# lucidrains/naturalspeech2-pytorch

Measured on NVIDIA H100. Metric: denoiser-steps/sec, higher is better.
Workload: dtype bf16

## Files before the change

naturalspeech2_pytorch_b200/csrc/attn.cu:

```cuda
#include "ptx.cuh"
#include "philox.cuh"
#include "host_common.h"
#include "../../include/ns2_b200.h"

namespace ns2 {

namespace attn {
constexpr int BQ = 128;
constexpr int BKV = 128;
constexpr int DH = 64;
constexpr int KVS = 3;
constexpr int Q_BYTES = BQ * DH * 2;
constexpr int KV_BYTES = BKV * DH * 2;
constexpr int OFF_Q = 0;
constexpr int OFF_K = OFF_Q + Q_BYTES;
constexpr int OFF_V = OFF_K + KVS * KV_BYTES;
constexpr int OFF_BAR = OFF_V + KVS * KV_BYTES;
constexpr int SMEM_BYTES = OFF_BAR + 256;
constexpr int THREADS = 384;
}

struct AttnDev {
  CUtensorMap tmQ, tmK, tmV;
  __nv_bfloat16* out;
  long long o_rs, o_bs;
  int q_len, kv_len;
  float scale_log2e;
  float* lse;
  DropoutDev drop;
  const int* kv_lens;
};

__device__ __forceinline__ float ex2_approx(float x) {
  float y;
  asm("ex2.approx.ftz.f32 %0, %1;" : "=f"(y) : "f"(x));
  return y;
}

__device__ __forceinline__ float keep_if(float x, uint32_t bits, int n) { return (bits >> n) & 1u ? x : 0.f; }

template <bool DROPOUT, bool RAGGED>
__global__ void __launch_bounds__(attn::THREADS, 1) attn_fwd_kernel(const __grid_constant__ AttnDev p) {
  static_assert(!(DROPOUT && RAGGED), "no dropout variant of the key-padding kernel");
  using namespace attn;
  extern __shared__ __align__(1024) uint8_t smem[];
  uint64_t* bars = reinterpret_cast<uint64_t*>(smem + OFF_BAR);
  uint64_t* q_full = bars + 0;
  uint64_t* kv_full = bars + 1;
  uint64_t* kv_empty = bars + 1 + KVS;

  const int warp = threadIdx.x >> 5, lane = threadIdx.x & 31;
  const int q0 = blockIdx.x * BQ;
  const int head = blockIdx.y;
  const int b = blockIdx.z;
  const int kv_len_b = RAGGED ? min(max(__ldg(p.kv_lens + b), 1), p.kv_len) : 0;
#define NS2_ATTN_KV_LEN (RAGGED ? kv_len_b : p.kv_len)
  const int T = (NS2_ATTN_KV_LEN + BKV - 1) / BKV;

  if (threadIdx.x == 0) {
    if ((smem_u32(smem) & 1023u) != 0) __trap();
    tma_prefetch_desc(&p.tmQ);
    tma_prefetch_desc(&p.tmK);
    tma_prefetch_desc(&p.tmV);
    mbar_init(smem_u32(q_full), 1);
    for (int i = 0; i < KVS; ++i) {
      mbar_init(smem_u32(&kv_full[i]), 1);
      mbar_init(smem_u32(&kv_empty[i]), 8);
    }
    fence_barrier_init();
  }
  __syncthreads();

  if (warp < 4) {
    asm volatile("setmaxnreg.dec.sync.aligned.u32 40;");
    if (warp == 0 && lane == 0) {
      mbar_arrive_expect_tx(smem_u32(q_full), Q_BYTES);
      tma_load_3d(smem_u32(smem + OFF_Q), &p.tmQ, smem_u32(q_full), head * DH, q0, b);
      for (int j = 0; j < T; ++j) {
        const int st = j % KVS;
        const uint32_t ph = (j / KVS) & 1;
        mbar_wait(smem_u32(&kv_empty[st]), ph ^ 1);
        const uint32_t fb = smem_u32(&kv_full[st]);
        mbar_arrive_expect_tx(fb, 2 * KV_BYTES);
        tma_load_3d(smem_u32(smem + OFF_K + st * KV_BYTES), &p.tmK, fb, head * DH, j * BKV, b);
        tma_load_3d(smem_u32(smem + OFF_V + st * KV_BYTES), &p.tmV, fb, head * DH, j * BKV, b);
      }
    }
  } else {
    asm volatile("setmaxnreg.inc.sync.aligned.u32 232;");
    const int w = (warp >> 2) - 1;
    const int r0 = 64 * w + 16 * (warp & 3) + (lane >> 2);
    const int c2 = 2 * (lane & 3);
    const float c = p.scale_log2e;
    float o_acc[DH / 2];
#pragma unroll
    for (int i = 0; i < DH / 2; ++i) o_acc[i] = 0.f;
    float m_run[2] = {-INFINITY, -INFINITY}, l_run[2] = {0.f, 0.f};
    const uint64_t dq = gmma_desc_sw128(smem_u32(smem + OFF_Q + w * (64 * 128)), 16, 1024);
    mbar_wait(smem_u32(q_full), 0);

    for (int j = 0; j < T; ++j) {
      const int st = j % KVS;
      mbar_wait(smem_u32(&kv_full[st]), (j / KVS) & 1);
      float s[BKV / 2];
      uint32_t keep[2];
      {
        const uint64_t dk = gmma_desc_sw128(smem_u32(smem + OFF_K + st * KV_BYTES), 16, 1024);
        wgmma_fence();
#pragma unroll
        for (int k = 0; k < DH / 16; ++k) wgmma_bf16_ss_n128<0, 0>(s, dq + 2 * k, dk + 2 * k, k > 0 ? 1u : 0u);
        wgmma_commit();
        if constexpr (DROPOUT) {
          const uint32_t cq = philox_attn_index(q0 + r0), cbh = b * gridDim.y + head, th = p.drop.threshold;
#pragma unroll
          for (int h = 0; h < 2; ++h) {
            keep[h] = 0u;
#pragma unroll 1
            for (int kk = 0; kk < 4; ++kk)
#pragma unroll
              for (int t = 0; t < 2; ++t) {
                const Philox4 r = philox4x32_10(philox_attn_index(j * BKV + 16 * (4 * h + kk) + c2 + t), cq, cbh,
                                                p.drop.site, p.drop.key0, p.drop.key1);
                const int n = 8 * kk + t;
                keep[h] |= (r.x >= th ? 1u : 0u) << n | (r.y >= th ? 1u : 0u) << (n + 4) |
                           (r.z >= th ? 1u : 0u) << (n + 2) | (r.w >= th ? 1u : 0u) << (n + 6);
              }
          }
        }
        wgmma_wait<0>();
        wgmma_hold(s);
      }
      const int valid = NS2_ATTN_KV_LEN - j * BKV;
      if (valid < BKV) {
#pragma unroll
        for (int jj = 0; jj < BKV / 8; ++jj)
#pragma unroll
          for (int e = 0; e < 4; ++e)
            if (8 * jj + c2 + (e & 1) >= valid) s[4 * jj + e] = -INFINITY;
      }
      float a[2], m_new[2];
#pragma unroll
      for (int i = 0; i < 2; ++i) {
        float m = -INFINITY;
#pragma unroll
        for (int jj = 0; jj < BKV / 8; ++jj) m = fmaxf(m, fmaxf(s[4 * jj + 2 * i], s[4 * jj + 2 * i + 1]));
        m = fmaxf(m, __shfl_xor_sync(0xffffffffu, m, 1));
        m = fmaxf(m, __shfl_xor_sync(0xffffffffu, m, 2));
        m_new[i] = fmaxf(m_run[i], m * c);
        a[i] = ex2_approx(m_run[i] - m_new[i]);
        m_run[i] = m_new[i];
        l_run[i] *= a[i];
      }
#pragma unroll
      for (int jj = 0; jj < DH / 8; ++jj) {
        o_acc[4 * jj + 0] *= a[0];
        o_acc[4 * jj + 1] *= a[0];
        o_acc[4 * jj + 2] *= a[1];
        o_acc[4 * jj + 3] *= a[1];
      }
      uint32_t pa[BKV / 16][4];
#pragma unroll
      for (int jj = 0; jj < BKV / 8; ++jj) {
        const float p0 = ex2_approx(fmaf(s[4 * jj + 0], c, -m_new[0]));
        const float p1 = ex2_approx(fmaf(s[4 * jj + 1], c, -m_new[0]));
        const float p2 = ex2_approx(fmaf(s[4 * jj + 2], c, -m_new[1]));
        const float p3 = ex2_approx(fmaf(s[4 * jj + 3], c, -m_new[1]));
        l_run[0] += p0 + p1;
        l_run[1] += p2 + p3;
        if constexpr (DROPOUT) {
          const uint32_t kb = keep[jj >> 3];
          const int n = (4 * jj) & 31;
          pa[jj >> 1][(jj & 1) * 2 + 0] = pack_bf16x2(keep_if(p0, kb, n), keep_if(p1, kb, n + 1));
          pa[jj >> 1][(jj & 1) * 2 + 1] = pack_bf16x2(keep_if(p2, kb, n + 2), keep_if(p3, kb, n + 3));
        } else {
          pa[jj >> 1][(jj & 1) * 2 + 0] = pack_bf16x2(p0, p1);
          pa[jj >> 1][(jj & 1) * 2 + 1] = pack_bf16x2(p2, p3);
        }
      }
      {
        const uint32_t vbase = smem_u32(smem + OFF_V + st * KV_BYTES);
        wgmma_fence();
#pragma unroll
        for (int k = 0; k < BKV / 16; ++k)
          wgmma_bf16_rs_n64<1>(o_acc, pa[k], gmma_desc_sw128(vbase + k * 2048, 1024, 1024), 1u);
        wgmma_commit();
        wgmma_wait<0>();
        wgmma_hold(o_acc);
      }
      __syncwarp();
      if (lane == 0) mbar_arrive(smem_u32(&kv_empty[st]));
    }

#pragma unroll
    for (int i = 0; i < 2; ++i) {
      float l = l_run[i];
      l += __shfl_xor_sync(0xffffffffu, l, 1);
      l += __shfl_xor_sync(0xffffffffu, l, 2);
      const int qrow = q0 + r0 + 8 * i;
      if (qrow < p.q_len) {
        const float inv = DROPOUT ? p.drop.scale / l : 1.0f / l;
        if (p.lse != nullptr && (lane & 3) == 0)
          p.lse[(static_cast<long long>(b) * gridDim.y + head) * p.q_len + qrow] = m_run[i] + log2f(l);
        __nv_bfloat16* op = p.out + static_cast<long long>(b) * p.o_bs + static_cast<long long>(qrow) * p.o_rs +
                            head * DH + c2;
#pragma unroll
        for (int jj = 0; jj < DH / 8; ++jj)
          *reinterpret_cast<uint32_t*>(op + 8 * jj) =
              pack_bf16x2(o_acc[4 * jj + 2 * i] * inv, o_acc[4 * jj + 2 * i + 1] * inv);
      }
    }
  }
#undef NS2_ATTN_KV_LEN
}

}

using namespace ns2;

extern "C" int ns2_attn_fwd(const ns2_attn_args* a, ns2_stream_t stream_) {
  NS2_REQUIRE(a != nullptr, "attn_fwd: NULL args");
  const ns2_dropout* d = a->dropout;
  DropoutDev drop;
  NS2_REQUIRE(d == nullptr || make_dropout_dev(d->seed, d->site, d->p, &drop), "attn_fwd: dropout p=%g is not in [0, 1)",
              static_cast<double>(d->p));
  const bool dropout = d != nullptr && d->p != 0.0f;
  NS2_REQUIRE(!(dropout && a->kv_lens), "attn_fwd: kv_lens with dropout p > 0 is not supported");
  NS2_REQUIRE(a->q && a->k && a->v && a->out, "attn_fwd: NULL pointer");
  NS2_REQUIRE(a->dim_head == 64, "attn_fwd: dim_head=%d, only 64 is supported", a->dim_head);
  NS2_REQUIRE(a->batches > 0 && a->heads > 0 && a->q_len > 0 && a->kv_len > 0, "attn_fwd: empty problem");
  NS2_REQUIRE(a->o_row_stride % 8 == 0 && a->o_batch_stride % 8 == 0 &&
                  (reinterpret_cast<uintptr_t>(a->out) & 15) == 0,
              "attn_fwd: out must be 16-byte aligned with strides multiple of 8");
  const cudaStream_t stream = static_cast<cudaStream_t>(stream_);
  AttnDev dev;
  memset(&dev, 0, sizeof(dev));
  const uint32_t box[3] = {64, attn::BQ, 1};
  const uint32_t box_kv[3] = {64, attn::BKV, 1};
  {
    const uint64_t dims[3] = {(uint64_t)a->heads * 64, (uint64_t)a->q_len, (uint64_t)a->batches};
    const uint64_t str[3] = {2, (uint64_t)a->q_row_stride * 2, (uint64_t)a->q_batch_stride * 2};
    int rc = make_tmap_16bit(&dev.tmQ, a->q, 3, dims, str, box);
    if (rc != kOk) return rc;
  }
  {
    const uint64_t dims[3] = {(uint64_t)a->heads * 64, (uint64_t)a->kv_len, (uint64_t)a->batches};
    const uint64_t strk[3] = {2, (uint64_t)a->k_row_stride * 2, (uint64_t)a->k_batch_stride * 2};
    const uint64_t strv[3] = {2, (uint64_t)a->v_row_stride * 2, (uint64_t)a->v_batch_stride * 2};
    int rc = make_tmap_16bit(&dev.tmK, a->k, 3, dims, strk, box_kv);
    if (rc != kOk) return rc;
    rc = make_tmap_16bit(&dev.tmV, a->v, 3, dims, strv, box_kv);
    if (rc != kOk) return rc;
  }
  dev.out = reinterpret_cast<__nv_bfloat16*>(a->out);
  dev.o_rs = a->o_row_stride;
  dev.o_bs = a->o_batch_stride;
  dev.q_len = a->q_len;
  dev.kv_len = a->kv_len;
  dev.scale_log2e = a->scale * 1.4426950408889634f;
  dev.lse = a->lse;
  dim3 grid((a->q_len + attn::BQ - 1) / attn::BQ, a->heads, a->batches);
  if (a->kv_lens != nullptr) {
    dev.kv_lens = a->kv_lens;
    NS2_CUDA_CHECK(set_max_smem_once(attn_fwd_kernel<false, true>, attn::SMEM_BYTES));
    attn_fwd_kernel<false, true><<<grid, attn::THREADS, attn::SMEM_BYTES, stream>>>(dev);
  } else if (!dropout) {
    NS2_CUDA_CHECK(set_max_smem_once(attn_fwd_kernel<false, false>, attn::SMEM_BYTES));
    attn_fwd_kernel<false, false><<<grid, attn::THREADS, attn::SMEM_BYTES, stream>>>(dev);
  } else {
    dev.drop = drop;
    NS2_CUDA_CHECK(set_max_smem_once(attn_fwd_kernel<true, false>, attn::SMEM_BYTES));
    attn_fwd_kernel<true, false><<<grid, attn::THREADS, attn::SMEM_BYTES, stream>>>(dev);
  }
  return launched(1);
}
```

Before: 65.78.

## Make attention forward kernel persistent with cross-tile Q/KV prefetch

Turns the flash-attention forward kernel into a persistent kernel: the grid is capped at the SM count and each CTA loops over (q-tile, head, batch) work items. The producer warp keeps a global KV stage counter so the K/V ring buffer carries across tiles, and a new q_empty barrier lets it load the next Q tile once consumers finish their last QK^T. This is meant to hide per-CTA launch, prologue and tail latency and to overlap the next tile's loads with the current tile's epilogue. In exchange the item-to-CTA mapping is static round-robin, which can leave tail imbalance when items have uneven KV lengths.

New measurement: 66.50, median of 6. 1.01x the previous value.

```diff
diff --git a/naturalspeech2_pytorch_b200/csrc/attn.cu b/naturalspeech2_pytorch_b200/csrc/attn.cu
--- a/naturalspeech2_pytorch_b200/csrc/attn.cu
+++ b/naturalspeech2_pytorch_b200/csrc/attn.cu
@@ -25,6 +25,7 @@
   __nv_bfloat16* out;
   long long o_rs, o_bs;
   int q_len, kv_len;
+  int q_tiles, heads, num_items;
   float scale_log2e;
   float* lse;
   DropoutDev drop;
@@ -48,14 +49,18 @@
   uint64_t* q_full = bars + 0;
   uint64_t* kv_full = bars + 1;
   uint64_t* kv_empty = bars + 1 + KVS;
+  uint64_t* q_empty = bars + 1 + 2 * KVS;
 
   const int warp = threadIdx.x >> 5, lane = threadIdx.x & 31;
-  const int q0 = blockIdx.x * BQ;
-  const int head = blockIdx.y;
-  const int b = blockIdx.z;
-  const int kv_len_b = RAGGED ? min(max(__ldg(p.kv_lens + b), 1), p.kv_len) : 0;
+  int q0, head, b, kv_len_b, T;
+  auto item = [&](int it) {
+    q0 = (it % p.q_tiles) * BQ;
+    head = (it / p.q_tiles) % p.heads;
+    b = it / (p.q_tiles * p.heads);
+    kv_len_b = RAGGED ? min(max(__ldg(p.kv_lens + b), 1), p.kv_len) : 0;
+    T = ((RAGGED ? kv_len_b : p.kv_len) + BKV - 1) / BKV;
+  };
 #define NS2_ATTN_KV_LEN (RAGGED ? kv_len_b : p.kv_len)
-  const int T = (NS2_ATTN_KV_LEN + BKV - 1) / BKV;
 
   if (threadIdx.x == 0) {
     if ((smem_u32(smem) & 1023u) != 0) __trap();
@@ -67,6 +72,7 @@
       mbar_init(smem_u32(&kv_full[i]), 1);
       mbar_init(smem_u32(&kv_empty[i]), 8);
     }
+    mbar_init(smem_u32(q_empty), 8);
     fence_barrier_init();
   }
   __syncthreads();
@@ -74,16 +80,21 @@
   if (warp < 4) {
     asm volatile("setmaxnreg.dec.sync.aligned.u32 40;");
     if (warp == 0 && lane == 0) {
-      mbar_arrive_expect_tx(smem_u32(q_full), Q_BYTES);
-      tma_load_3d(smem_u32(smem + OFF_Q), &p.tmQ, smem_u32(q_full), head * DH, q0, b);
-      for (int j = 0; j < T; ++j) {
-        const int st = j % KVS;
-        const uint32_t ph = (j / KVS) & 1;
-        mbar_wait(smem_u32(&kv_empty[st]), ph ^ 1);
-        const uint32_t fb = smem_u32(&kv_full[st]);
-        mbar_arrive_expect_tx(fb, 2 * KV_BYTES);
-        tma_load_3d(smem_u32(smem + OFF_K + st * KV_BYTES), &p.tmK, fb, head * DH, j * BKV, b);
-        tma_load_3d(smem_u32(smem + OFF_V + st * KV_BYTES), &p.tmV, fb, head * DH, j * BKV, b);
+      uint32_t n = 0, kt = 0;
+      for (int it = blockIdx.x; it < p.num_items; it += gridDim.x, ++n) {
+        item(it);
+        mbar_wait(smem_u32(q_empty), (n & 1) ^ 1);
+        mbar_arrive_expect_tx(smem_u32(q_full), Q_BYTES);
+        tma_load_3d(smem_u32(smem + OFF_Q), &p.tmQ, smem_u32(q_full), head * DH, q0, b);
+        for (int j = 0; j < T; ++j, ++kt) {
+          const int st = kt % KVS;
+          const uint32_t ph = (kt / KVS) & 1;
+          mbar_wait(smem_u32(&kv_empty[st]), ph ^ 1);
+          const uint32_t fb = smem_u32(&kv_full[st]);
+          mbar_arrive_expect_tx(fb, 2 * KV_BYTES);
+          tma_load_3d(smem_u32(smem + OFF_K + st * KV_BYTES), &p.tmK, fb, head * DH, j * BKV, b);
+          tma_load_3d(smem_u32(smem + OFF_V + st * KV_BYTES), &p.tmV, fb, head * DH, j * BKV, b);
+        }
       }
     }
   } else {
@@ -92,121 +103,129 @@
     const int r0 = 64 * w + 16 * (warp & 3) + (lane >> 2);
     const int c2 = 2 * (lane & 3);
     const float c = p.scale_log2e;
-    float o_acc[DH / 2];
-#pragma unroll
-    for (int i = 0; i < DH / 2; ++i) o_acc[i] = 0.f;
-    float m_run[2] = {-INFINITY, -INFINITY}, l_run[2] = {0.f, 0.f};
     const uint64_t dq = gmma_desc_sw128(smem_u32(smem + OFF_Q + w * (64 * 128)), 16, 1024);
-    mbar_wait(smem_u32(q_full), 0);
-
-    for (int j = 0; j < T; ++j) {
-      const int st = j % KVS;
-      mbar_wait(smem_u32(&kv_full[st]), (j / KVS) & 1);
-      float s[BKV / 2];
-      uint32_t keep[2];
-      {
-        const uint64_t dk = gmma_desc_sw128(smem_u32(smem + OFF_K + st * KV_BYTES), 16, 1024);
-        wgmma_fence();
-#pragma unroll
-        for (int k = 0; k < DH / 16; ++k) wgmma_bf16_ss_n128<0, 0>(s, dq + 2 * k, dk + 2 * k, k > 0 ? 1u : 0u);
-        wgmma_commit();
-        if constexpr (DROPOUT) {
-          const uint32_t cq = philox_attn_index(q0 + r0), cbh = b * gridDim.y + head, th = p.drop.threshold;
-#pragma unroll
-          for (int h = 0; h < 2; ++h) {
-            keep[h] = 0u;
+    uint32_t n = 0, kt = 0;
+    for (int it = blockIdx.x; it < p.num_items; it += gridDim.x, ++n) {
+      item(it);
+      float o_acc[DH / 2];
+#pragma unroll
+      for (int i = 0; i < DH / 2; ++i) o_acc[i] = 0.f;
+      float m_run[2] = {-INFINITY, -INFINITY}, l_run[2] = {0.f, 0.f};
+      mbar_wait(smem_u32(q_full), n & 1);
+
+      for (int j = 0; j < T; ++j, ++kt) {
+        const int st = kt % KVS;
+        mbar_wait(smem_u32(&kv_full[st]), (kt / KVS) & 1);
+        float s[BKV / 2];
+        uint32_t keep[2];
+        {
+          const uint64_t dk = gmma_desc_sw128(smem_u32(smem + OFF_K + st * KV_BYTES), 16, 1024);
+          wgmma_fence();
+#pragma unroll
+          for (int k = 0; k < DH / 16; ++k) wgmma_bf16_ss_n128<0, 0>(s, dq + 2 * k, dk + 2 * k, k > 0 ? 1u : 0u);
+          wgmma_commit();
+          if constexpr (DROPOUT) {
+            const uint32_t cq = philox_attn_index(q0 + r0), cbh = b * p.heads + head, th = p.drop.threshold;
+#pragma unroll
+            for (int h = 0; h < 2; ++h) {
+              keep[h] = 0u;
 #pragma unroll 1
-            for (int kk = 0; kk < 4; ++kk)
-#pragma unroll
-              for (int t = 0; t < 2; ++t) {
-                const Philox4 r = philox4x32_10(philox_attn_index(j * BKV + 16 * (4 * h + kk) + c2 + t), cq, cbh,
-                                                p.drop.site, p.drop.key0, p.drop.key1);
-                const int n = 8 * kk + t;
-                keep[h] |= (r.x >= th ? 1u : 0u) << n | (r.y >= th ? 1u : 0u) << (n + 4) |
-                           (r.z >= th ? 1u : 0u) << (n + 2) | (r.w >= th ? 1u : 0u) << (n + 6);
-              }
+              for (int kk = 0; kk < 4; ++kk)
+#pragma unroll
+                for (int t = 0; t < 2; ++t) {
+                  const Philox4 r = philox4x32_10(philox_attn_index(j * BKV + 16 * (4 * h + kk) + c2 + t), cq, cbh,
+                                                  p.drop.site, p.drop.key0, p.drop.key1);
+                  const int n = 8 * kk + t;
+                  keep[h] |= (r.x >= th ? 1u : 0u) << n | (r.y >= th ? 1u : 0u) << (n + 4) |
+                             (r.z >= th ? 1u : 0u) << (n + 2) | (r.w >= th ? 1u : 0u) << (n + 6);
+                }
+            }
           }
-        }
-        wgmma_wait<0>();
-        wgmma_hold(s);
+          wgmma_wait<0>();
+          wgmma_hold(s);
+        }
+        if (j == T - 1) {
+          __syncwarp();
+          if (lane == 0) mbar_arrive(smem_u32(q_empty));
+        }
+        const int valid = NS2_ATTN_KV_LEN - j * BKV;
+        if (valid < BKV) {
+#pragma unroll
+          for (int jj = 0; jj < BKV / 8; ++jj)
+#pragma unroll
+            for (int e = 0; e < 4; ++e)
+              if (8 * jj + c2 + (e & 1) >= valid) s[4 * jj + e] = -INFINITY;
+        }
+        float a[2], m_new[2];
+#pragma unroll
+        for (int i = 0; i < 2; ++i) {
+          float m = -INFINITY;
+#pragma unroll
+          for (int jj = 0; jj < BKV / 8; ++jj) m = fmaxf(m, fmaxf(s[4 * jj + 2 * i], s[4 * jj + 2 * i + 1]));
+          m = fmaxf(m, __shfl_xor_sync(0xffffffffu, m, 1));
+          m = fmaxf(m, __shfl_xor_sync(0xffffffffu, m, 2));
+          m_new[i] = fmaxf(m_run[i], m * c);
+          a[i] = ex2_approx(m_run[i] - m_new[i]);
+          m_run[i] = m_new[i];
+          l_run[i] *= a[i];
+        }
+#pragma unroll
+        for (int jj = 0; jj < DH / 8; ++jj) {
+          o_acc[4 * jj + 0] *= a[0];
+          o_acc[4 * jj + 1] *= a[0];
+          o_acc[4 * jj + 2] *= a[1];
+          o_acc[4 * jj + 3] *= a[1];
+        }
+        uint32_t pa[BKV / 16][4];
+#pragma unroll
+        for (int jj = 0; jj < BKV / 8; ++jj) {
+          const float p0 = ex2_approx(fmaf(s[4 * jj + 0], c, -m_new[0]));
+          const float p1 = ex2_approx(fmaf(s[4 * jj + 1], c, -m_new[0]));
+          const float p2 = ex2_approx(fmaf(s[4 * jj + 2], c, -m_new[1]));
+          const float p3 = ex2_approx(fmaf(s[4 * jj + 3], c, -m_new[1]));
+          l_run[0] += p0 + p1;
+          l_run[1] += p2 + p3;
+          if constexpr (DROPOUT) {
+            const uint32_t kb = keep[jj >> 3];
+            const int n = (4 * jj) & 31;
+            pa[jj >> 1][(jj & 1) * 2 + 0] = pack_bf16x2(keep_if(p0, kb, n), keep_if(p1, kb, n + 1));
+            pa[jj >> 1][(jj & 1) * 2 + 1] = pack_bf16x2(keep_if(p2, kb, n + 2), keep_if(p3, kb, n + 3));
+          } else {
+            pa[jj >> 1][(jj & 1) * 2 + 0] = pack_bf16x2(p0, p1);
+            pa[jj >> 1][(jj & 1) * 2 + 1] = pack_bf16x2(p2, p3);
+          }
+        }
+        {
+          const uint32_t vbase = smem_u32(smem + OFF_V + st * KV_BYTES);
+          wgmma_fence();
+#pragma unroll
+          for (int k = 0; k < BKV / 16; ++k)
+            wgmma_bf16_rs_n64<1>(o_acc, pa[k], gmma_desc_sw128(vbase + k * 2048, 1024, 1024), 1u);
+          wgmma_commit();
+          wgmma_wait<0>();
+          wgmma_hold(o_acc);
+        }
+        __syncwarp();
+        if (lane == 0) mbar_arrive(smem_u32(&kv_empty[st]));
       }
-      const int valid = NS2_ATTN_KV_LEN - j * BKV;
-      if (valid < BKV) {
-#pragma unroll
-        for (int jj = 0; jj < BKV / 8; ++jj)
-#pragma unroll
-          for (int e = 0; e < 4; ++e)
-            if (8 * jj + c2 + (e & 1) >= valid) s[4 * jj + e] = -INFINITY;
-      }
-      float a[2], m_new[2];
+
 #pragma unroll
       for (int i = 0; i < 2; ++i) {
-        float m = -INFINITY;
-#pragma unroll
-        for (int jj = 0; jj < BKV / 8; ++jj) m = fmaxf(m, fmaxf(s[4 * jj + 2 * i], s[4 * jj + 2 * i + 1]));
-        m = fmaxf(m, __shfl_xor_sync(0xffffffffu, m, 1));
-        m = fmaxf(m, __shfl_xor_sync(0xffffffffu, m, 2));
-        m_new[i] = fmaxf(m_run[i], m * c);
-        a[i] = ex2_approx(m_run[i] - m_new[i]);
-        m_run[i] = m_new[i];
-        l_run[i] *= a[i];
-      }
-#pragma unroll
-      for (int jj = 0; jj < DH / 8; ++jj) {
-        o_acc[4 * jj + 0] *= a[0];
-        o_acc[4 * jj + 1] *= a[0];
-        o_acc[4 * jj + 2] *= a[1];
-        o_acc[4 * jj + 3] *= a[1];
-      }
-      uint32_t pa[BKV / 16][4];
-#pragma unroll
-      for (int jj = 0; jj < BKV / 8; ++jj) {
-        const float p0 = ex2_approx(fmaf(s[4 * jj + 0], c, -m_new[0]));
-        const float p1 = ex2_approx(fmaf(s[4 * jj + 1], c, -m_new[0]));
-        const float p2 = ex2_approx(fmaf(s[4 * jj + 2], c, -m_new[1]));
-        const float p3 = ex2_approx(fmaf(s[4 * jj + 3], c, -m_new[1]));
-        l_run[0] += p0 + p1;
-        l_run[1] += p2 + p3;
-        if constexpr (DROPOUT) {
-          const uint32_t kb = keep[jj >> 3];
-          const int n = (4 * jj) & 31;
-          pa[jj >> 1][(jj & 1) * 2 + 0] = pack_bf16x2(keep_if(p0, kb, n), keep_if(p1, kb, n + 1));
-          pa[jj >> 1][(jj & 1) * 2 + 1] = pack_bf16x2(keep_if(p2, kb, n + 2), keep_if(p3, kb, n + 3));
-        } else {
-          pa[jj >> 1][(jj & 1) * 2 + 0] = pack_bf16x2(p0, p1);
-          pa[jj >> 1][(jj & 1) * 2 + 1] = pack_bf16x2(p2, p3);
-        }
-      }
-      {
-        const uint32_t vbase = smem_u32(smem + OFF_V + st * KV_BYTES);
-        wgmma_fence();
-#pragma unroll
-        for (int k = 0; k < BKV / 16; ++k)
-          wgmma_bf16_rs_n64<1>(o_acc, pa[k], gmma_desc_sw128(vbase + k * 2048, 1024, 1024), 1u);
-        wgmma_commit();
-        wgmma_wait<0>();
-        wgmma_hold(o_acc);
-      }
-      __syncwarp();
-      if (lane == 0) mbar_arrive(smem_u32(&kv_empty[st]));
-    }
-
-#pragma unroll
-    for (int i = 0; i < 2; ++i) {
-      float l = l_run[i];
-      l += __shfl_xor_sync(0xffffffffu, l, 1);
-      l += __shfl_xor_sync(0xffffffffu, l, 2);
-      const int qrow = q0 + r0 + 8 * i;
-      if (qrow < p.q_len) {
-        const float inv = DROPOUT ? p.drop.scale / l : 1.0f / l;
-        if (p.lse != nullptr && (lane & 3) == 0)
-          p.lse[(static_cast<long long>(b) * gridDim.y + head) * p.q_len + qrow] = m_run[i] + log2f(l);
-        __nv_bfloat16* op = p.out + static_cast<long long>(b) * p.o_bs + static_cast<long long>(qrow) * p.o_rs +
-                            head * DH + c2;
-#pragma unroll
-        for (int jj = 0; jj < DH / 8; ++jj)
-          *reinterpret_cast<uint32_t*>(op + 8 * jj) =
-              pack_bf16x2(o_acc[4 * jj + 2 * i] * inv, o_acc[4 * jj + 2 * i + 1] * inv);
+        float l = l_run[i];
+        l += __shfl_xor_sync(0xffffffffu, l, 1);
+        l += __shfl_xor_sync(0xffffffffu, l, 2);
+        const int qrow = q0 + r0 + 8 * i;
+        if (qrow < p.q_len) {
+          const float inv = DROPOUT ? p.drop.scale / l : 1.0f / l;
+          if (p.lse != nullptr && (lane & 3) == 0)
+            p.lse[(static_cast<long long>(b) * p.heads + head) * p.q_len + qrow] = m_run[i] + log2f(l);
+          __nv_bfloat16* op = p.out + static_cast<long long>(b) * p.o_bs + static_cast<long long>(qrow) * p.o_rs +
+                              head * DH + c2;
+#pragma unroll
+          for (int jj = 0; jj < DH / 8; ++jj)
+            *reinterpret_cast<uint32_t*>(op + 8 * jj) =
+                pack_bf16x2(o_acc[4 * jj + 2 * i] * inv, o_acc[4 * jj + 2 * i + 1] * inv);
+        }
       }
     }
   }
@@ -258,7 +277,11 @@
   dev.kv_len = a->kv_len;
   dev.scale_log2e = a->scale * 1.4426950408889634f;
   dev.lse = a->lse;
-  dim3 grid((a->q_len + attn::BQ - 1) / attn::BQ, a->heads, a->batches);
+  dev.q_tiles = (a->q_len + attn::BQ - 1) / attn::BQ;
+  dev.heads = a->heads;
+  NS2_REQUIRE(static_cast<long long>(dev.q_tiles) * a->heads * a->batches <= INT32_MAX, "attn_fwd: too many tiles");
+  dev.num_items = dev.q_tiles * a->heads * a->batches;
+  const int grid = dev.num_items < num_sms() ? dev.num_items : num_sms();
   if (a->kv_lens != nullptr) {
     dev.kv_lens = a->kv_lens;
     NS2_CUDA_CHECK(set_max_smem_once(attn_fwd_kernel<false, true>, attn::SMEM_BYTES));
```

## Make attention kernel persistent with ping-pong warpgroups and overlapped PV GEMM

Applied to the files above, without the earlier changes.

Turns the attention forward kernel into a persistent kernel launched with one CTA per SM that loops over query tiles. The producer now double-buffers Q tiles and uses four KV stages. The two consumer warpgroups take turns on the tensor cores through named barriers. Each iteration issues the previous block's P·V wgmma together with the current QK^T wgmma, so one warpgroup's softmax can overlap the other's matrix work. This adds synchronisation complexity, more shared memory, and register pressure from carrying P across iterations.

Measured after the change: 65.81 before, 66.91 after (median of 6 runs). +1.7%, better.

```diff
diff --git a/naturalspeech2_pytorch_b200/csrc/attn.cu b/naturalspeech2_pytorch_b200/csrc/attn.cu
--- a/naturalspeech2_pytorch_b200/csrc/attn.cu
+++ b/naturalspeech2_pytorch_b200/csrc/attn.cu
@@ -9,15 +9,17 @@
 constexpr int BQ = 128;
 constexpr int BKV = 128;
 constexpr int DH = 64;
-constexpr int KVS = 3;
+constexpr int KVS = 4;
+constexpr int QS = 2;
 constexpr int Q_BYTES = BQ * DH * 2;
 constexpr int KV_BYTES = BKV * DH * 2;
 constexpr int OFF_Q = 0;
-constexpr int OFF_K = OFF_Q + Q_BYTES;
+constexpr int OFF_K = OFF_Q + QS * Q_BYTES;
 constexpr int OFF_V = OFF_K + KVS * KV_BYTES;
 constexpr int OFF_BAR = OFF_V + KVS * KV_BYTES;
 constexpr int SMEM_BYTES = OFF_BAR + 256;
 constexpr int THREADS = 384;
+constexpr int TURN_BAR = 1;
 }
 
 struct AttnDev {
@@ -25,6 +27,7 @@
   __nv_bfloat16* out;
   long long o_rs, o_bs;
   int q_len, kv_len;
+  int q_tiles, heads, batches;
   float scale_log2e;
   float* lse;
   DropoutDev drop;
@@ -38,6 +41,22 @@
 }
 
 __device__ __forceinline__ float keep_if(float x, uint32_t bits, int n) { return (bits >> n) & 1u ? x : 0.f; }
+
+template <int ID>
+__device__ __forceinline__ void turn_sync() {
+  asm volatile("bar.sync %0, 256;" ::"n"(ID) : "memory");
+}
+template <int ID>
+__device__ __forceinline__ void turn_arrive() {
+  asm volatile("bar.arrive %0, 256;" ::"n"(ID) : "memory");
+}
+
+__device__ __forceinline__ void issue_pv(float (&o_acc)[attn::DH / 2], const uint32_t (&pa)[attn::BKV / 16][4],
+                                         uint32_t vbase) {
+#pragma unroll
+  for (int k = 0; k < attn::BKV / 16; ++k)
+    wgmma_bf16_rs_n64<1>(o_acc, pa[k], gmma_desc_sw128(vbase + k * 2048, 1024, 1024), 1u);
+}
 
 template <bool DROPOUT, bool RAGGED>
 __global__ void __launch_bounds__(attn::THREADS, 1) attn_fwd_kernel(const __grid_constant__ AttnDev p) {
@@ -46,23 +65,32 @@
   extern __shared__ __align__(1024) uint8_t smem[];
   uint64_t* bars = reinterpret_cast<uint64_t*>(smem + OFF_BAR);
   uint64_t* q_full = bars + 0;
-  uint64_t* kv_full = bars + 1;
-  uint64_t* kv_empty = bars + 1 + KVS;
+  uint64_t* q_empty = bars + QS;
+  uint64_t* kv_full = bars + 2 * QS;
+  uint64_t* kv_empty = bars + 2 * QS + KVS;
 
   const int warp = threadIdx.x >> 5, lane = threadIdx.x & 31;
-  const int q0 = blockIdx.x * BQ;
-  const int head = blockIdx.y;
-  const int b = blockIdx.z;
-  const int kv_len_b = RAGGED ? min(max(__ldg(p.kv_lens + b), 1), p.kv_len) : 0;
-#define NS2_ATTN_KV_LEN (RAGGED ? kv_len_b : p.kv_len)
-  const int T = (NS2_ATTN_KV_LEN + BKV - 1) / BKV;
+  const int tiles = p.q_tiles * p.heads * p.batches;
+  struct Item { int q0, head, b, kv_len, T; };
+  const auto item = [&](int t) {
+    Item it;
+    it.q0 = (t % p.q_tiles) * BQ;
+    it.head = (t / p.q_tiles) % p.heads;
+    it.b = t / (p.q_tiles * p.heads);
+    it.kv_len = RAGGED ? min(max(__ldg(p.kv_lens + it.b), 1), p.kv_len) : p.kv_len;
+    it.T = (it.kv_len + BKV - 1) / BKV;
+    return it;
+  };
 
   if (threadIdx.x == 0) {
     if ((smem_u32(smem) & 1023u) != 0) __trap();
     tma_prefetch_desc(&p.tmQ);
     tma_prefetch_desc(&p.tmK);
     tma_prefetch_desc(&p.tmV);
-    mbar_init(smem_u32(q_full), 1);
+    for (int i = 0; i < QS; ++i) {
+      mbar_init(smem_u32(&q_full[i]), 1);
+      mbar_init(smem_u32(&q_empty[i]), 8);
+    }
     for (int i = 0; i < KVS; ++i) {
       mbar_init(smem_u32(&kv_full[i]), 1);
       mbar_init(smem_u32(&kv_empty[i]), 8);
@@ -74,16 +102,21 @@
   if (warp < 4) {
     asm volatile("setmaxnreg.dec.sync.aligned.u32 40;");
     if (warp == 0 && lane == 0) {
-      mbar_arrive_expect_tx(smem_u32(q_full), Q_BYTES);
-      tma_load_3d(smem_u32(smem + OFF_Q), &p.tmQ, smem_u32(q_full), head * DH, q0, b);
-      for (int j = 0; j < T; ++j) {
-        const int st = j % KVS;
-        const uint32_t ph = (j / KVS) & 1;
-        mbar_wait(smem_u32(&kv_empty[st]), ph ^ 1);
-        const uint32_t fb = smem_u32(&kv_full[st]);
-        mbar_arrive_expect_tx(fb, 2 * KV_BYTES);
-        tma_load_3d(smem_u32(smem + OFF_K + st * KV_BYTES), &p.tmK, fb, head * DH, j * BKV, b);
-        tma_load_3d(smem_u32(smem + OFF_V + st * KV_BYTES), &p.tmV, fb, head * DH, j * BKV, b);
+      int g = 0;
+      for (int t = blockIdx.x, n = 0; t < tiles; t += gridDim.x, ++n) {
+        const Item it = item(t);
+        const int qs = n % QS;
+        mbar_wait(smem_u32(&q_empty[qs]), ((n / QS) & 1) ^ 1);
+        mbar_arrive_expect_tx(smem_u32(&q_full[qs]), Q_BYTES);
+        tma_load_3d(smem_u32(smem + OFF_Q + qs * Q_BYTES), &p.tmQ, smem_u32(&q_full[qs]), it.head * DH, it.q0, it.b);
+        for (int j = 0; j < it.T; ++j, ++g) {
+          const int st = g % KVS;
+          mbar_wait(smem_u32(&kv_empty[st]), ((g / KVS) & 1) ^ 1);
+          const uint32_t fb = smem_u32(&kv_full[st]);
+          mbar_arrive_expect_tx(fb, 2 * KV_BYTES);
+          tma_load_3d(smem_u32(smem + OFF_K + st * KV_BYTES), &p.tmK, fb, it.head * DH, j * BKV, it.b);
+          tma_load_3d(smem_u32(smem + OFF_V + st * KV_BYTES), &p.tmV, fb, it.head * DH, j * BKV, it.b);
+        }
       }
     }
   } else {
@@ -92,125 +125,148 @@
     const int r0 = 64 * w + 16 * (warp & 3) + (lane >> 2);
     const int c2 = 2 * (lane & 3);
     const float c = p.scale_log2e;
-    float o_acc[DH / 2];
-#pragma unroll
-    for (int i = 0; i < DH / 2; ++i) o_acc[i] = 0.f;
-    float m_run[2] = {-INFINITY, -INFINITY}, l_run[2] = {0.f, 0.f};
-    const uint64_t dq = gmma_desc_sw128(smem_u32(smem + OFF_Q + w * (64 * 128)), 16, 1024);
-    mbar_wait(smem_u32(q_full), 0);
-
-    for (int j = 0; j < T; ++j) {
-      const int st = j % KVS;
-      mbar_wait(smem_u32(&kv_full[st]), (j / KVS) & 1);
-      float s[BKV / 2];
-      uint32_t keep[2];
-      {
-        const uint64_t dk = gmma_desc_sw128(smem_u32(smem + OFF_K + st * KV_BYTES), 16, 1024);
-        wgmma_fence();
-#pragma unroll
-        for (int k = 0; k < DH / 16; ++k) wgmma_bf16_ss_n128<0, 0>(s, dq + 2 * k, dk + 2 * k, k > 0 ? 1u : 0u);
-        wgmma_commit();
-        if constexpr (DROPOUT) {
-          const uint32_t cq = philox_attn_index(q0 + r0), cbh = b * gridDim.y + head, th = p.drop.threshold;
-#pragma unroll
-          for (int h = 0; h < 2; ++h) {
-            keep[h] = 0u;
+
+    const auto sync_own = [&] { w == 0 ? turn_sync<TURN_BAR + 0>() : turn_sync<TURN_BAR + 1>(); };
+    const auto arrive_other = [&] { w == 0 ? turn_arrive<TURN_BAR + 1>() : turn_arrive<TURN_BAR + 0>(); };
+    if (w == 1) turn_arrive<TURN_BAR + 0>();
+
+    int g = 0;
+    for (int t = blockIdx.x, n = 0; t < tiles; t += gridDim.x, ++n) {
+      const Item it = item(t);
+      const int q0 = it.q0, head = it.head, b = it.b, T = it.T;
+      const int qs = n % QS;
+      float o_acc[DH / 2];
+#pragma unroll
+      for (int i = 0; i < DH / 2; ++i) o_acc[i] = 0.f;
+      float m_run[2] = {-INFINITY, -INFINITY}, l_run[2] = {0.f, 0.f};
+      const uint64_t dq = gmma_desc_sw128(smem_u32(smem + OFF_Q + qs * Q_BYTES + w * (64 * 128)), 16, 1024);
+      uint32_t pa[BKV / 16][4];
+      mbar_wait(smem_u32(&q_full[qs]), (n / QS) & 1);
+
+      for (int j = 0; j < T; ++j) {
+        const int st = (g + j) % KVS;
+        const int st_prev = (g + j + KVS - 1) % KVS;
+        mbar_wait(smem_u32(&kv_full[st]), ((g + j) / KVS) & 1);
+        float s[BKV / 2];
+        uint32_t keep[2];
+        {
+          const uint64_t dk = gmma_desc_sw128(smem_u32(smem + OFF_K + st * KV_BYTES), 16, 1024);
+          sync_own();
+          wgmma_fence();
+          if (j > 0) issue_pv(o_acc, pa, smem_u32(smem + OFF_V + st_prev * KV_BYTES));
+#pragma unroll
+          for (int k = 0; k < DH / 16; ++k) wgmma_bf16_ss_n128<0, 0>(s, dq + 2 * k, dk + 2 * k, k > 0 ? 1u : 0u);
+          wgmma_commit();
+          arrive_other();
+          if constexpr (DROPOUT) {
+            const uint32_t cq = philox_attn_index(q0 + r0), cbh = b * p.heads + head, th = p.drop.threshold;
+#pragma unroll
+            for (int h = 0; h < 2; ++h) {
+              keep[h] = 0u;
 #pragma unroll 1
-            for (int kk = 0; kk < 4; ++kk)
-#pragma unroll
-              for (int t = 0; t < 2; ++t) {
-                const Philox4 r = philox4x32_10(philox_attn_index(j * BKV + 16 * (4 * h + kk) + c2 + t), cq, cbh,
-                                                p.drop.site, p.drop.key0, p.drop.key1);
-                const int n = 8 * kk + t;
-                keep[h] |= (r.x >= th ? 1u : 0u) << n | (r.y >= th ? 1u : 0u) << (n + 4) |
-                           (r.z >= th ? 1u : 0u) << (n + 2) | (r.w >= th ? 1u : 0u) << (n + 6);
-              }
+              for (int kk = 0; kk < 4; ++kk)
+#pragma unroll
+                for (int tt = 0; tt < 2; ++tt) {
+                  const Philox4 r = philox4x32_10(philox_attn_index(j * BKV + 16 * (4 * h + kk) + c2 + tt), cq, cbh,
+                                                  p.drop.site, p.drop.key0, p.drop.key1);
+                  const int e = 8 * kk + tt;
+                  keep[h] |= (r.x >= th ? 1u : 0u) << e | (r.y >= th ? 1u : 0u) << (e + 4) |
+                             (r.z >= th ? 1u : 0u) << (e + 2) | (r.w >= th ? 1u : 0u) << (e + 6);
+                }
+            }
           }
-        }
-        wgmma_wait<0>();
-        wgmma_hold(s);
-      }
-      const int valid = NS2_ATTN_KV_LEN - j * BKV;
-      if (valid < BKV) {
-#pragma unroll
-        for (int jj = 0; jj < BKV / 8; ++jj)
-#pragma unroll
-          for (int e = 0; e < 4; ++e)
-            if (8 * jj + c2 + (e & 1) >= valid) s[4 * jj + e] = -INFINITY;
-      }
-      float a[2], m_new[2];
-#pragma unroll
-      for (int i = 0; i < 2; ++i) {
-        float m = -INFINITY;
-#pragma unroll
-        for (int jj = 0; jj < BKV / 8; ++jj) m = fmaxf(m, fmaxf(s[4 * jj + 2 * i], s[4 * jj + 2 * i + 1]));
-        m = fmaxf(m, __shfl_xor_sync(0xffffffffu, m, 1));
-        m = fmaxf(m, __shfl_xor_sync(0xffffffffu, m, 2));
-        m_new[i] = fmaxf(m_run[i], m * c);
-        a[i] = ex2_approx(m_run[i] - m_new[i]);
-        m_run[i] = m_new[i];
-        l_run[i] *= a[i];
-      }
-#pragma unroll
-      for (int jj = 0; jj < DH / 8; ++jj) {
-        o_acc[4 * jj + 0] *= a[0];
-        o_acc[4 * jj + 1] *= a[0];
-        o_acc[4 * jj + 2] *= a[1];
-        o_acc[4 * jj + 3] *= a[1];
-      }
-      uint32_t pa[BKV / 16][4];
-#pragma unroll
-      for (int jj = 0; jj < BKV / 8; ++jj) {
-        const float p0 = ex2_approx(fmaf(s[4 * jj + 0], c, -m_new[0]));
-        const float p1 = ex2_approx(fmaf(s[4 * jj + 1], c, -m_new[0]));
-        const float p2 = ex2_approx(fmaf(s[4 * jj + 2], c, -m_new[1]));
-        const float p3 = ex2_approx(fmaf(s[4 * jj + 3], c, -m_new[1]));
-        l_run[0] += p0 + p1;
-        l_run[1] += p2 + p3;
-        if constexpr (DROPOUT) {
-          const uint32_t kb = keep[jj >> 3];
-          const int n = (4 * jj) & 31;
-          pa[jj >> 1][(jj & 1) * 2 + 0] = pack_bf16x2(keep_if(p0, kb, n), keep_if(p1, kb, n + 1));
-          pa[jj >> 1][(jj & 1) * 2 + 1] = pack_bf16x2(keep_if(p2, kb, n + 2), keep_if(p3, kb, n + 3));
-        } else {
-          pa[jj >> 1][(jj & 1) * 2 + 0] = pack_bf16x2(p0, p1);
-          pa[jj >> 1][(jj & 1) * 2 + 1] = pack_bf16x2(p2, p3);
+          wgmma_wait<0>();
+          wgmma_hold(s);
+          wgmma_hold(o_acc);
+        }
+        if (j > 0 || j == T - 1) {
+          __syncwarp();
+          if (lane == 0) {
+            if (j > 0) mbar_arrive(smem_u32(&kv_empty[st_prev]));
+            if (j == T - 1) mbar_arrive(smem_u32(&q_empty[qs]));
+          }
+        }
+        const int valid = it.kv_len - j * BKV;
+        if (valid < BKV) {
+#pragma unroll
+          for (int jj = 0; jj < BKV / 8; ++jj)
+#pragma unroll
+            for (int e = 0; e < 4; ++e)
+              if (8 * jj + c2 + (e & 1) >= valid) s[4 * jj + e] = -INFINITY;
+        }
+        float a[2], m_new[2];
+#pragma unroll
+        for (int i = 0; i < 2; ++i) {
+          float m = -INFINITY;
+#pragma unroll
+          for (int jj = 0; jj < BKV / 8; ++jj) m = fmaxf(m, fmaxf(s[4 * jj + 2 * i], s[4 * jj + 2 * i + 1]));
+          m = fmaxf(m, __shfl_xor_sync(0xffffffffu, m, 1));
+          m = fmaxf(m, __shfl_xor_sync(0xffffffffu, m, 2));
+          m_new[i] = fmaxf(m_run[i], m * c);
+          a[i] = ex2_approx(m_run[i] - m_new[i]);
+          m_run[i] = m_new[i];
+          l_run[i] *= a[i];
+        }
+#pragma unroll
+        for (int jj = 0; jj < DH / 8; ++jj) {
+          o_acc[4 * jj + 0] *= a[0];
+          o_acc[4 * jj + 1] *= a[0];
+          o_acc[4 * jj + 2] *= a[1];
+          o_acc[4 * jj + 3] *= a[1];
+        }
+#pragma unroll
+        for (int jj = 0; jj < BKV / 8; ++jj) {
+          const float p0 = ex2_approx(fmaf(s[4 * jj + 0], c, -m_new[0]));
+          const float p1 = ex2_approx(fmaf(s[4 * jj + 1], c, -m_new[0]));
+          const float p2 = ex2_approx(fmaf(s[4 * jj + 2], c, -m_new[1]));
+          const float p3 = ex2_approx(fmaf(s[4 * jj + 3], c, -m_new[1]));
+          l_run[0] += p0 + p1;
+          l_run[1] += p2 + p3;
+          if constexpr (DROPOUT) {
+            const uint32_t kb = keep[jj >> 3];
+            const int e = (4 * jj) & 31;
+            pa[jj >> 1][(jj & 1) * 2 + 0] = pack_bf16x2(keep_if(p0, kb, e), keep_if(p1, kb, e + 1));
+            pa[jj >> 1][(jj & 1) * 2 + 1] = pack_bf16x2(keep_if(p2, kb, e + 2), keep_if(p3, kb, e + 3));
+          } else {
+            pa[jj >> 1][(jj & 1) * 2 + 0] = pack_bf16x2(p0, p1);
+            pa[jj >> 1][(jj & 1) * 2 + 1] = pack_bf16x2(p2, p3);
+          }
         }
       }
       {
-        const uint32_t vbase = smem_u32(smem + OFF_V + st * KV_BYTES);
+        const int st_last = (g + T - 1) % KVS;
+        sync_own();
         wgmma_fence();
-#pragma unroll
-        for (int k = 0; k < BKV / 16; ++k)
-          wgmma_bf16_rs_n64<1>(o_acc, pa[k], gmma_desc_sw128(vbase + k * 2048, 1024, 1024), 1u);
+        issue_pv(o_acc, pa, smem_u32(smem + OFF_V + st_last * KV_BYTES));
         wgmma_commit();
+        if (w == 0 || t + static_cast<int>(gridDim.x) < tiles) arrive_other();
         wgmma_wait<0>();
         wgmma_hold(o_acc);
+        __syncwarp();
+        if (lane == 0) mbar_arrive(smem_u32(&kv_empty[st_last]));
       }
-      __syncwarp();
-      if (lane == 0) mbar_arrive(smem_u32(&kv_empty[st]));
-    }
-
-#pragma unroll
-    for (int i = 0; i < 2; ++i) {
-      float l = l_run[i];
-      l += __shfl_xor_sync(0xffffffffu, l, 1);
-      l += __shfl_xor_sync(0xffffffffu, l, 2);
-      const int qrow = q0 + r0 + 8 * i;
-      if (qrow < p.q_len) {
-        const float inv = DROPOUT ? p.drop.scale / l : 1.0f / l;
-        if (p.lse != nullptr && (lane & 3) == 0)
-          p.lse[(static_cast<long long>(b) * gridDim.y + head) * p.q_len + qrow] = m_run[i] + log2f(l);
-        __nv_bfloat16* op = p.out + static_cast<long long>(b) * p.o_bs + static_cast<long long>(qrow) * p.o_rs +
-                            head * DH + c2;
-#pragma unroll
-        for (int jj = 0; jj < DH / 8; ++jj)
-          *reinterpret_cast<uint32_t*>(op + 8 * jj) =
-              pack_bf16x2(o_acc[4 * jj + 2 * i] * inv, o_acc[4 * jj + 2 * i + 1] * inv);
+      g += T;
+
+#pragma unroll
+      for (int i = 0; i < 2; ++i) {
+        float l = l_run[i];
+        l += __shfl_xor_sync(0xffffffffu, l, 1);
+        l += __shfl_xor_sync(0xffffffffu, l, 2);
+        const int qrow = q0 + r0 + 8 * i;
+        if (qrow < p.q_len) {
+          const float inv = DROPOUT ? p.drop.scale / l : 1.0f / l;
+          if (p.lse != nullptr && (lane & 3) == 0)
+            p.lse[(static_cast<long long>(b) * p.heads + head) * p.q_len + qrow] = m_run[i] + log2f(l);
+          __nv_bfloat16* op = p.out + static_cast<long long>(b) * p.o_bs + static_cast<long long>(qrow) * p.o_rs +
+                              head * DH + c2;
+#pragma unroll
+          for (int jj = 0; jj < DH / 8; ++jj)
+            *reinterpret_cast<uint32_t*>(op + 8 * jj) =
+                pack_bf16x2(o_acc[4 * jj + 2 * i] * inv, o_acc[4 * jj + 2 * i + 1] * inv);
+        }
       }
     }
   }
-#undef NS2_ATTN_KV_LEN
 }
 
 }
@@ -258,7 +314,12 @@
   dev.kv_len = a->kv_len;
   dev.scale_log2e = a->scale * 1.4426950408889634f;
   dev.lse = a->lse;
-  dim3 grid((a->q_len + attn::BQ - 1) / attn::BQ, a->heads, a->batches);
+  dev.q_tiles = (a->q_len + attn::BQ - 1) / attn::BQ;
+  dev.heads = a->heads;
+  dev.batches = a->batches;
+  const long long tiles = static_cast<long long>(dev.q_tiles) * a->heads * a->batches;
+  NS2_REQUIRE(tiles <= INT_MAX, "attn_fwd: %lld query tiles", tiles);
+  const dim3 grid(static_cast<unsigned>(tiles < num_sms() ? tiles : num_sms()));
   if (a->kv_lens != nullptr) {
     dev.kv_lens = a->kv_lens;
     NS2_CUDA_CHECK(set_max_smem_once(attn_fwd_kernel<false, true>, attn::SMEM_BYTES));
```
